# silversixpence-crypto/zk-proof-of-assets

Hardware: AMD Instinct MI355X
Metric: G1-MSM throughput (higher is better)
Workload: dtype u32x8 (254-bit modular integer); 1 GPU; BN254 G1 Pippenger MSM, 2^20 points per GPU, uniform 252-bit scalars, bases (a+i*b)*G resident in HBM (BASELINE.json configs[1]); points_per_gpu=1048576, msms_in_flight=6, form=classic: arbitrary bases, nothing precomputed, checked=not in a plain run (--full checks the known discrete log)

## Files before the change

zk-proof-of-assets_amd/csrc/device_ctx.hpp:

```cpp
#pragma once
#include <hip/hip_runtime.h>
#include <stdint.h>
#include <stdio.h>
#include <stdlib.h>
#include <time.h>
#include <atomic>
#include <condition_variable>
#include <string.h>
#include <exception>
#include <functional>
#include <mutex>
#include <stdexcept>
#include <thread>
#include <string>
#include <vector>

namespace zkpoa {

struct HipError : std::runtime_error {
  explicit HipError(const std::string& s) : std::runtime_error(s) {}
};

struct OomError : HipError {
  explicit OomError(const std::string& s) : HipError(s) {}
// ... 37 lines not shown
    ZK_HIP(e);
    cap = bytes;
  }
  void reset() { off = 0; }
  template <class T>
  T* take(size_t count) {
    size_t bytes = (count * sizeof(T) + 255) & ~size_t(255);
    if (off + bytes > cap) throw HipError("arena overflow (reserve() too small)");
    T* p = reinterpret_cast<T*>(base + off);
    off += bytes;
    return p;
  }
  void release() {
    if (base) (void)hipFree(base);
    base = nullptr;
    cap = off = 0;
  }
};

struct Lane {
  hipStream_t stream = nullptr;
  Arena ws;
  void* pinned = nullptr;
  void* pinned_dev = nullptr;
  size_t pinned_cap = 0;
  std::vector<char> host_sums;
  hipEvent_t ev0 = nullptr, ev1 = nullptr;
  void* scan_scratch = nullptr;
  uint32_t scan_tiles = 0, scan_gen = 0;
  uint32_t scan_poll_limit = 1u << 24, scan_test_withhold = 0;
  static constexpr size_t kFaultBytes = 64;
  volatile uint32_t* fault_word() const { return reinterpret_cast<volatile uint32_t*>(static_cast<char*>(pinned) + pinned_cap); }
  uint32_t* fault_word_dev() const { return reinterpret_cast<uint32_t*>(static_cast<char*>(pinned_dev) + pinned_cap); }
  void init(int level = 0) {
    int lo = 0, hi = 0;
    ZK_HIP(hipDeviceGetStreamPriorityRange(&lo, &hi));
    int prio = level >= 2 ? hi : (level == 1 ? (lo + hi) / 2 : lo);
    ZK_HIP(hipStreamCreateWithPriority(&stream, hipStreamNonBlocking, prio));
    pinned_cap = (1 << 20) - kFaultBytes;
    ZK_HIP(hipHostMalloc(&pinned, pinned_cap + kFaultBytes, hipHostMallocDefault));
    ZK_HIP(hipHostGetDevicePointer(&pinned_dev, pinned, 0));
    memset(static_cast<char*>(pinned) + pinned_cap, 0, kFaultBytes);
    host_sums.assign(pinned_cap + kFaultBytes, 0);
    ZK_HIP(hipEventCreate(&ev0));
    ZK_HIP(hipEventCreate(&ev1));
  }
  void destroy() {
    ws.release();
    if (scan_scratch) (void)hipFree(scan_scratch);
    scan_scratch = nullptr;
    scan_tiles = scan_gen = 0;
    if (pinned) (void)hipHostFree(pinned);
    if (stream) (void)hipStreamDestroy(stream);
    if (ev0) (void)hipEventDestroy(ev0);
    if (ev1) (void)hipEventDestroy(ev1);
    pinned = nullptr;
    stream = nullptr;
    ev0 = ev1 = nullptr;
  }
};

struct DeviceCtx {
  int device = 0;
  int num_cu = 256;
  static constexpr int kLanes = 12;
  static constexpr int kEagerLanes = 5;
  Lane lanes[kLanes];
  std::mutex lazy_mutex_;
  bool ok = false;
  float last_ms[8] = {0, 0, 0, 0, 0, 0, 0, 0};
  std::thread bg_;
  std::mutex bg_mutex_;
  std::condition_variable bg_cv_;
  bool lanes_ready_ = false;
  std::exception_ptr bg_err_;
  hipStream_t copy_stream = nullptr;
  std::function<void(hipStream_t)> after_copy_stream;
  std::function<void()> after_lanes;
  std::mutex copy_mutex_;
  std::condition_variable copy_cv_;
  bool copy_done_ = false;

  void init(int dev) {
    const bool verbose = getenv("ZKPOA_VERBOSE") != nullptr;
    auto now_ms = [] {
      struct timespec ts;
      clock_gettime(CLOCK_MONOTONIC, &ts);
      return ts.tv_sec * 1e3 + ts.tv_nsec / 1e6;
    };
    double t0 = now_ms();
    int count = 0;
// ... 101 lines not shown
```

zk-proof-of-assets_amd/csrc/msm.hip.h:

```cpp
#pragma once
#include "bn254_ec.hip.h"
#include "fq29.hip.h"
#include "device_ctx.hpp"
#include "msm_plan.hpp"
#include <string.h>
#include <chrono>
#include <utility>

namespace zkpoa {

__device__ static const uint32_t kHalfR[8] = {0xf8000000u, 0xa1f0fac9u, 0x3cdcb848u, 0x9419f424u,
                                              0x40c0ac2eu, 0xdc2822dbu, 0x7098d014u, 0x18322739u};

ZK_DEV bool scalar_normalize(uint32_t (&s)[8]) {
  uint32_t bw = 0;
#pragma unroll
  for (int i = 0; i < 8; i++) (void)subb(kHalfR[i], s[i], bw);
  if (!bw) return false;
  uint32_t b2 = 0;
#pragma unroll
  for (int i = 0; i < 8; i++) s[i] = subb(FrParams::P[i], s[i], b2);
  return true;
}

// ... 9 lines not shown
  s[0] = a.x; s[1] = a.y; s[2] = a.z; s[3] = a.w;
  s[4] = b.x; s[5] = b.y; s[6] = b.z; s[7] = b.w;
}

static __global__ __launch_bounds__(256) void msm_density_kernel(const void* __restrict__ scalars, uint64_t n,
                                                                 unsigned long long* __restrict__ out) {
  __shared__ unsigned int acc[kDensityHi - kDensityLo + 1];
  if (threadIdx.x <= (unsigned)(kDensityHi - kDensityLo)) acc[threadIdx.x] = 0;
  __syncthreads();
  uint64_t i = (uint64_t)blockIdx.x * 256u + threadIdx.x;
  uint32_t L = 0;
  if (i < n) {
    uint32_t s[8];
    const uint4* p = reinterpret_cast<const uint4*>(scalars) + 2 * i;
    uint4 a = p[0], b = p[1];
    s[0] = a.x; s[1] = a.y; s[2] = a.z; s[3] = a.w;
    s[4] = b.x; s[5] = b.y; s[6] = b.z; s[7] = b.w;
    (void)scalar_normalize(s);
#pragma unroll
    for (int k = 7; k >= 0; k--)
      if (L == 0 && s[k]) L = 32u * k + (32u - __builtin_clz(s[k]));
  }
  for (int c = kDensityLo; c <= kDensityHi; c++) {
    uint32_t d = (L + c - 1) / c;
#pragma unroll
    for (int o = 32; o > 0; o >>= 1) d += __shfl_xor(d, o);
    if ((threadIdx.x & 63u) == 0 && d) atomicAdd(&acc[c - kDensityLo], d);
  }
  __syncthreads();
  if (threadIdx.x <= (unsigned)(kDensityHi - kDensityLo) && acc[threadIdx.x])
    atomicAdd(&out[threadIdx.x], (unsigned long long)acc[threadIdx.x]);
}

ZK_DEV uint32_t scan_input(const uint32_t* __restrict__ in, uint32_t idx, uint32_t n, int mode, uint32_t K,
                           uint32_t& raw) {
  if (idx >= n) {
    raw = 0;
    return 0;
  }
  uint32_t x = in[idx];
  if (mode == 3) x = in[idx + 1] - x;
  raw = x;
  if (mode == 0) return x;
  if (mode == 3 && x <= 1) return 0;
  return (x + K - 1) / K;
}
constexpr int kScanBlock = 256;
constexpr int kScanItems = 8;
constexpr int kScanTile = kScanBlock * kScanItems;

ZK_DEV uint32_t block_exclusive_scan(uint32_t v, uint32_t* lds, uint32_t& total) {
  uint32_t lane = threadIdx.x & 63u, wave = threadIdx.x >> 6;
  uint32_t x = v;
#pragma unroll
  for (int o = 1; o < 64; o <<= 1) {
    uint32_t y = __shfl_up(x, o);
    if (lane >= (uint32_t)o) x += y;
  }
  if (lane == 63) lds[wave] = x;
  __syncthreads();
  uint32_t base = 0, tot = 0;
#pragma unroll
  for (int k = 0; k < kScanBlock / 64; k++) {
    uint32_t t = lds[k];
    if ((uint32_t)k < wave) base += t;
    tot += t;
  }
  __syncthreads();
  total = tot;
  return base + x - v;
}

static __global__ __launch_bounds__(kScanBlock) void scan_reduce_kernel(const uint32_t* __restrict__ in, uint32_t n, int mode,
                                                                 uint32_t K, uint32_t* __restrict__ block_sums,
                                                                 uint32_t* __restrict__ max_out) {
  __shared__ uint32_t lds[8];
  uint32_t base = blockIdx.x * kScanTile + threadIdx.x * kScanItems;
  uint32_t sum = 0, mx = 0;
// ... 137 lines not shown
  if (lane == 0) scan_status_store(&status[tile], tag2 | (running + aggregate));
  return running;
}

static __global__ __launch_bounds__(kScanBlock) void scan_pair_kernel(ScanPair a, uint64_t* __restrict__ status_a,
                                                                      uint64_t* __restrict__ status_b,
                                                                      uint32_t* __restrict__ tickets, uint32_t gen,
                                                                      uint32_t ntiles, ScanGuard guard) {
  __shared__ uint32_t lds[8];
  __shared__ uint32_t s_tile, s_pre_a, s_pre_b;
  __shared__ uint32_t s_hist[kMaxPieceLenPlan + 1];
  if (threadIdx.x == 0) s_tile = atomicAdd(&tickets[0], 1u);
  if (a.hist)
    for (uint32_t i = threadIdx.x; i <= a.hist_K; i += kScanBlock) s_hist[i] = 0;
  __syncthreads();
  const uint32_t tile = s_tile;
  const uint32_t base = tile * kScanTile + threadIdx.x * kScanItems;
  const bool two = a.mode_b >= 0;
  uint32_t va[kScanItems], vb[kScanItems];
  uint32_t sum_a = 0, sum_b = 0, mx = 0;
#pragma unroll
  for (int k = 0; k < kScanItems; k++) {
    uint32_t raw;
    va[k] = scan_input(a.in, base + k, a.n, a.mode_a, a.K_a, raw);
    sum_a += va[k];
    mx = raw > mx ? raw : mx;
    if (a.hist && raw) {
      const uint32_t full = raw / a.hist_K, rem = raw - full * a.hist_K;
      if (full) atomicAdd(&s_hist[a.hist_K], full);
      if (rem) atomicAdd(&s_hist[rem], 1u);
    }
    vb[k] = 0;
    if (two) {
      if (a.mode_b == 0) vb[k] = raw;
      else if (a.mode_b == 3 && raw <= 1) vb[k] = 0;
      else vb[k] = (raw + a.K_b - 1) / a.K_b;
      sum_b += vb[k];
    }
  }
  uint32_t tot_a, tot_b = 0;
  uint32_t ex_a = block_exclusive_scan(sum_a, lds, tot_a);
  uint32_t ex_b = two ? block_exclusive_scan(sum_b, lds, tot_b) : 0;
  if (threadIdx.x < 64) {
    uint32_t pa = scan_look_back(status_a, tile, tot_a, gen, guard);
    uint32_t pb = two ? scan_look_back(status_b, tile, tot_b, gen, guard) : 0;
    if (threadIdx.x == 0) {
      s_pre_a = pa;
      s_pre_b = pb;
    }
  }
  __syncthreads();
  ex_a += s_pre_a;
  ex_b += s_pre_b;
#pragma unroll
  for (int k = 0; k < kScanItems; k++) {
    const uint32_t idx = base + k;
    if (idx < a.n) {
      a.out_a[idx] = ex_a;
      if (two) a.out_b[idx] = ex_b;
    }
    ex_a += va[k];
    ex_b += vb[k];
  }
  if (tile == ntiles - 1 && threadIdx.x == kScanBlock - 1) {
    a.out_a[a.n] = ex_a;
    if (a.total_a) *a.total_a = ex_a;
    if (two) {
      a.out_b[a.n] = ex_b;
      if (a.total_b) *a.total_b = ex_b;
// ... 69 lines not shown
ZK_DEV uint32_t find_bucket(const uint32_t* __restrict__ po, uint32_t nb, uint32_t t) {
  uint32_t lo = 0, hi = nb;
  while (hi - lo > 1) {
    uint32_t mid = (lo + hi) >> 1;
    if (po[mid] <= t) lo = mid; else hi = mid;
  }
  return lo;
}

}
#include "msm_sort.hip.h"
namespace zkpoa {

constexpr uint32_t kMaxPieceLen = 512;
static_assert(kMaxPieceLen == kMaxPieceLenPlan, "the plan, the scans' LDS histogram and the piece ordering share one bound");

constexpr uint32_t kPiecesPerThread = 8;
static __global__ __launch_bounds__(256) void msm_piece_hist_kernel(const uint32_t* __restrict__ cnt0, uint32_t TB,
                                                                    uint32_t K0, uint32_t* __restrict__ len_hist) {
  __shared__ uint32_t h[kMaxPieceLen + 1];
  for (uint32_t i = threadIdx.x; i <= K0; i += 256u) h[i] = 0;
  __syncthreads();
  const uint32_t b = blockIdx.x * 256u + threadIdx.x;
  const uint32_t x = b < TB ? cnt0[b] : 0u;
  if (x) {
    const uint32_t full = x / K0, rem = x - full * K0;
    if (full) atomicAdd(&h[K0], full);
    if (rem) atomicAdd(&h[rem], 1u);
  }
  __syncthreads();
  for (uint32_t i = threadIdx.x; i <= K0; i += 256u)
    if (h[i]) atomicAdd(&len_hist[i], h[i]);
}
static __global__ __launch_bounds__(256) void msm_piece_order_kernel(const uint32_t* __restrict__ cnt0,
                                                                     const uint32_t* __restrict__ po1, uint32_t TB,
                                                                     uint32_t K0, const uint32_t* __restrict__ len_hist,
                                                                     uint32_t* __restrict__ cursor,
                                                                     uint32_t* __restrict__ pbkt,
                                                                     uint32_t* __restrict__ order) {
  __shared__ uint32_t base[kMaxPieceLen + 2];
  __shared__ uint32_t h[kMaxPieceLen + 1];
  __shared__ uint32_t wsum[4];
  uint32_t tid = threadIdx.x;
  uint32_t v0 = 0, v1 = 0, v2 = 0;
  uint32_t r0 = 3 * tid, r1 = 3 * tid + 1, r2 = 3 * tid + 2;
  if (r0 <= kMaxPieceLen) v0 = len_hist[kMaxPieceLen - r0];
  if (r1 <= kMaxPieceLen) v1 = len_hist[kMaxPieceLen - r1];
  if (r2 <= kMaxPieceLen) v2 = len_hist[kMaxPieceLen - r2];
  uint32_t tot;
  uint32_t ex = block_exclusive_scan(v0 + v1 + v2, wsum, tot);
  if (r0 <= kMaxPieceLen) base[kMaxPieceLen - r0] = ex;
  if (r1 <= kMaxPieceLen) base[kMaxPieceLen - r1] = ex + v0;
  if (r2 <= kMaxPieceLen) base[kMaxPieceLen - r2] = ex + v0 + v1;
  for (uint32_t i = tid; i <= kMaxPieceLen; i += 256u) h[i] = 0;
  __syncthreads();
  const uint32_t total = po1[TB];
  uint32_t len[kPiecesPerThread], local[kPiecesPerThread];
#pragma unroll
  for (uint32_t k = 0; k < kPiecesPerThread; k++) {
    const uint32_t t = (blockIdx.x * kPiecesPerThread + k) * 256u + tid;
    len[k] = 0;
    local[k] = 0;
    if (t < total) {
      const uint32_t b = find_bucket(po1, TB, t);
      const uint32_t j = t - po1[b];
      uint32_t l = cnt0[b] - j * K0;
      if (l > K0) l = K0;
      pbkt[t] = b;
      len[k] = l;
      local[k] = atomicAdd(&h[l], 1u);
    }
  }
  __syncthreads();
  for (uint32_t i = tid; i <= kMaxPieceLen; i += 256u) {
    uint32_t c = h[i];
    if (c) h[i] = atomicAdd(&cursor[i], c);
  }
  __syncthreads();
#pragma unroll
  for (uint32_t k = 0; k < kPiecesPerThread; k++) {
    const uint32_t t = (blockIdx.x * kPiecesPerThread + k) * 256u + tid;
    if (t < total) order[base[len[k]] + h[len[k]] + local[k]] = t;
  }
}

#if defined(ZKPOA_G1_LIMB32)
constexpr bool kG1Limb29 = false;
#else
constexpr bool kG1Limb29 = true;
#endif
ZK_DEV XYZZ<Fq> xyzz_from_words_3q(const uint32_t* w) {
  XYZZ<Fq> r;
#pragma unroll
  for (int i = 0; i < 8; i++) {
    r.x.l[i] = w[i];
    r.y.l[i] = w[8 + i];
    r.zz.l[i] = w[16 + i];
    r.zzz.l[i] = w[24 + i];
  }
  r.x = Fq::reduce_2p(r.x);
  r.y = Fq::reduce_2p(r.y);
  r.zz = Fq::reduce_2p(r.zz);
  r.zzz = Fq::reduce_2p(r.zzz);
  return r;
}
ZK_DEV bool g1piece29_result(const G1Piece29& s, XYZZ<Fq>& out) {
  uint32_t w[32];
  g1piece29_finish(s, w);
  out = xyzz_from_words_3q(w);
  return s.empty || !out.zz.is_zero();
}

struct G1Sum29 {
  Xyzz29S p;
  bool inf;
// ... 373 lines not shown
template <class F, bool Packed = false, bool WireOut = false>
static __global__ __launch_bounds__(64, kRedWaves<Packed>) void msm_bit_tree_sum_kernel(const void* __restrict__ X, uint32_t E,
                                                                     uint32_t logS, uint32_t logRows, uint32_t nbits,
                                                                     uint32_t S_out, void* __restrict__ Y) {
  extern __shared__ __attribute__((aligned(16))) char lds_raw[];
  const uint32_t g = blockIdx.y / nbits, b = blockIdx.y % nbits, grp = g & 1u;
  const uint32_t cnt = grp ? (1u << logS) : (1u << logRows);
  msm_tree_run<F, Packed, WireOut>(X, (size_t)g * E, cnt, grp, (int)b, Y, (size_t)blockIdx.y * S_out + blockIdx.x, lds_raw);
}
template <class F, bool Packed = false, bool WireOut = false>
static __global__ __launch_bounds__(64, kRedWaves<Packed>) void msm_tree_sum_kernel(const void* __restrict__ X, uint32_t S, uint32_t S_out,
                                                           void* __restrict__ Y) {
  extern __shared__ __attribute__((aligned(16))) char lds_raw[];
  const uint32_t w = blockIdx.y;
  msm_tree_run<F, Packed, WireOut>(X, (size_t)w * S, S, 0u, -1, Y, (size_t)w * S_out + blockIdx.x, lds_raw);
}

template <class F>
struct MsmSizes {
  static constexpr size_t kAffine = 2 * FieldBytes<F>::N;
  static constexpr size_t kXyzz = 4 * FieldBytes<F>::N;
};

static __global__ __launch_bounds__(256) void msm_to_host_kernel(const uint4* __restrict__ src, uint4* __restrict__ dst,
                                                                 uint32_t n16) {
  for (uint32_t i = blockIdx.x * 256u + threadIdx.x; i < n16; i += gridDim.x * 256u) dst[i] = src[i];
}
inline void msm_read_back(Lane& lane, const void* d_src, size_t bytes) {
  if (bytes > lane.pinned_cap) throw HipError("msm: read-back larger than the pinned staging area");
  const uint32_t n16 = (uint32_t)((bytes + 15) / 16);
  const uint32_t grid = n16 > 4096 ? 16u : (n16 + 255) / 256;
  hipLaunchKernelGGL(msm_to_host_kernel, dim3(grid ? grid : 1), dim3(256), 0, lane.stream, (const uint4*)d_src,
                     (uint4*)lane.pinned_dev, n16);
  ZK_HIP(hipStreamSynchronize(lane.stream));
  lane_check_fault(lane);
}

inline void lane_scan(Lane& lane, const ScanPair& a, uint32_t* block_sums) {
  if (!scan_three_kernel()) return scan_pair(lane, a);
  scan_u32(lane.stream, a.in, a.n, a.mode_a, a.K_a, a.out_a, block_sums, a.total_a, a.max_out);
  if (a.mode_b >= 0) scan_u32(lane.stream, a.in, a.n, a.mode_b, a.K_b, a.out_b, block_sums, a.total_b, nullptr);
  if (a.hist)
    hipLaunchKernelGGL(msm_piece_hist_kernel, dim3((a.n + 255) / 256), dim3(256), 0, lane.stream, a.in, a.n, a.hist_K, a.hist);
}

struct ArenaCount {
  size_t off = 0;
  template <class T> T* take(size_t count) { return off += (count * sizeof(T) + 255) & ~size_t(255), nullptr; }
};
template <class Layout>
inline size_t msm_layout_bytes(const MsmPlan& p) {
  ArenaCount count;
  Layout().carve(count, p);
  return count.off;
}
template <class Layout>
inline Layout msm_carve(Arena& ws, const MsmPlan& p) {
  Layout m;
  const size_t start = ws.off;
  m.carve(ws, p);
  if (ws.off - start != msm_layout_bytes<Layout>(p)) throw HipError("msm: internal: workspace layout and its size disagree");
  return m;
}
inline size_t msm_piece_cap(const MsmPlan& p) { return (size_t)p.n * p.W / p.K0 + p.TB + 1; }

struct MsmSortLayout {
// ... 47 lines not shown
  char* buckets = nullptr;
  char *P1 = nullptr, *P2 = nullptr;
  size_t p1_cap = 0, p2_cap = 0;
  char* X = nullptr;
  char *Y1 = nullptr, *Y2 = nullptr;
  template <class Taker>
  void carve(Taker& ws, const MsmPlan& p) {
    constexpr size_t kXyzz = MsmSizes<F>::kXyzz;
    const size_t E = (size_t)1 << p.logS, sums = (size_t)2 * p.Wb * msm_reduce_bits(p.logS);
    po_b = ws.template take<uint32_t>(p.TB + 1);
    po_c = ws.template take<uint32_t>(p.TB + 1);
    block_sums = ws.template take<uint32_t>(p.TB / kScanTile + 2);
    misc = ws.template take<uint32_t>(16);
    buckets = ws.template take<char>((size_t)p.TB * kXyzz);
    p1_cap = msm_piece_cap(p);
    p2_cap = p1_cap / 2 + 1;
    P1 = ws.template take<char>(p1_cap * kXyzz);
    P2 = ws.template take<char>(p2_cap * kXyzz);
    X = ws.template take<char>(2 * p.Wb * E * kXyzz);
    Y1 = ws.template take<char>((E + 255) / 256 * sums * kXyzz);
    Y2 = ws.template take<char>((E + 255) / 256 * sums * kXyzz);
  }
};

inline size_t msm_sort_workspace_bytes(const MsmPlan& p) { return msm_layout_bytes<MsmSortLayout>(p) + (1 << 12) - 256; }
template <class F>
inline size_t msm_accum_workspace_bytes(const MsmPlan& p) { return msm_layout_bytes<MsmAccumLayout<F>>(p) + (1 << 12); }

template <class F, bool Packed = false, class Scan>
inline void msm_reduce_levels(hipStream_t st, uint32_t TB, uint32_t K, const uint32_t* po_in, uint32_t* po_b,
                              uint32_t* po_c, char* Pin, size_t cap_in, char* Pout, size_t cap_out, uint64_t max_items,
                              uint64_t total_in, void* buckets, Scan scan) {
  uint32_t* po_out = po_b;
  while (max_items > 1) {
    uint64_t bound = total_in / 2 + 1;
    if (bound > cap_out) throw HipError("msm: level buffer too small");
    scan(po_in, po_out);
    hipLaunchKernelGGL((msm_accumN_kernel<F, Packed>), dim3((uint32_t)((bound + 255) / 256)), dim3(256), 0, st, (const void*)Pin,
                       po_in, (const uint32_t*)po_out, TB, K, buckets, (void*)Pout);
    max_items = (max_items + K - 1) / K;
    total_in = bound;
    po_in = po_out;
    po_out = (po_out == po_b) ? po_c : po_b;
    std::swap(Pin, Pout);
    std::swap(cap_in, cap_out);
  }
}

struct MsmSorted {
  MsmPlan p;
  MsmSortLayout m;
  uint32_t total1 = 0;
  uint32_t total_entries = 0;
  uint32_t max_count = 0;
};

inline void lane_reserve(Lane& lane, size_t need) {
  if (lane.ws.cap < need) {
    ZK_HIP(hipStreamSynchronize(lane.stream));
    const auto t0 = std::chrono::steady_clock::now();
    lane.ws.reserve(need);
    const double ms = std::chrono::duration<double, std::milli>(std::chrono::steady_clock::now() - t0).count();
    if (ms > 20.0 && getenv("ZKPOA_VERBOSE"))
      fprintf(stderr, "zkpoa:   lane workspace grows to %.2f GB: hipFree + hipMalloc %.1f ms\n", need / 1e9, ms);
  }
}

inline MsmSorted msm_sort_phase(Lane& lane, const void* d_scalars, const MsmRequest& req,
                                size_t (*extra)(const MsmPlan&), bool sync_at_end = false) {
  MsmSorted sr;
  sr.p = msm_make_plan(req);
  const MsmPlan& p = sr.p;
  if ((uint64_t)p.n * p.W + p.TB >= 0xffff0000ull) throw HipError("msm: n * windows exceeds the 32-bit entry index");
  if (p.merged && (uint64_t)p.n * p.W >= 0x80000000ull) throw HipError("msm: n * windows exceeds the fixed-base entry index");
  hipStream_t st = lane.stream;
  lane_reserve(lane, msm_sort_workspace_bytes(p) + (extra ? extra(p) : 0));
  lane.ws.reset();
  const SortPlan sp = make_sort_plan(p.ne, p.Wb, p.c);
  const MsmSortLayout& m = sr.m = msm_carve<MsmSortLayout>(lane.ws, p);
  ZK_HIP(hipMemsetAsync(m.counts, 0, m.zero_bytes, st));
  static const bool no_sparse = [] {
    const char* e = getenv("ZKPOA_NO_SPARSE");
    return e && *e == '1';
  }();
  const bool sparse = p.sparse && !no_sparse;
  uint32_t* digits = sparse ? nullptr : m.digits();
  uint2* elist = sparse ? m.elist : nullptr;
  uint32_t* pre = sparse ? m.pre : nullptr;
  const uint32_t nblk = (p.n + 255) / 256;
  if (p.n && !sparse) hipLaunchKernelGGL(msm_digits_kernel, dim3(nblk), dim3(256), 0, st, d_scalars, p.n, p.c, p.W, digits);
  if (sparse) {
    const uint32_t per_wg = kEntriesThreads * kEntriesPerThread;
    hipLaunchKernelGGL(msm_entries_kernel, dim3((p.n + per_wg - 1) / per_wg), dim3(kEntriesThreads), 0, st, d_scalars, p.n,
                       p.c, p.W, elist, m.misc + 8);
    hipLaunchKernelGGL(msm_entries_finish_kernel, dim3(1), dim3(1), 0, st, (const uint32_t*)(m.misc + 8), sp.CH, pre, pre + 4);
  }
  for (uint32_t l = 0; l < sp.npass; l++) {
    const bool first = l == 0 && !sparse, last = l + 1 == sp.npass;
    const uint2* in = l == 0 ? (const uint2*)elist : m.ebuf[(l - 1) & 1];
    uint2* out = last ? nullptr : m.ebuf[l & 1];
    const uint32_t* in_off = l == 0 ? (const uint32_t*)pre : m.seg_off[l - 1];
    const uint32_t* tpo = l == 0 ? (const uint32_t*)(pre ? pre + 4 : nullptr) : m.seg_tpo[l - 1];
    uint32_t* out_cnt = last ? m.counts : m.seg_cnt[l];
    uint32_t* out_off = last ? m.off0 : m.seg_off[l];
    const dim3 grid = first ? dim3(sp.chunks0, sp.W) : dim3((uint32_t)sp.tasks_max[l]);
    if (p.n) {
      if (first)
        hipLaunchKernelGGL((msm_sort_count_kernel<true>), grid, dim3(256), 0, st, sp, l, (const uint32_t*)digits, in,
                           in_off, tpo, out_cnt, m.base[l]);
      else
        hipLaunchKernelGGL((msm_sort_count_kernel<false>), grid, dim3(256), 0, st, sp, l, (const uint32_t*)digits, in,
                           in_off, tpo, out_cnt, m.base[l]);
    }
    lane_scan(lane,
              last ? ScanPair{m.counts, p.TB, 0, 0, m.off0, m.misc + 0, 1, p.K0, m.po_a, m.misc + 2, m.misc + 1, m.len_hist, p.K0}
                   : ScanPair{m.seg_cnt[l], sp.segs[l + 1], 0, 0, m.seg_off[l], m.misc + 4 + 2 * l, 1, sp.CH, m.seg_tpo[l],
                              m.misc + 5 + 2 * l, nullptr},
              m.block_sums);
    if (p.n) {
#define ZK_SORT_SCATTER(F_, L_)                                                                                       \
  hipLaunchKernelGGL((msm_sort_scatter_kernel<F_, L_>), grid, dim3(256), 0, st, sp, l, (const uint32_t*)digits, in,  \
                     in_off, tpo, (const uint32_t*)out_off, (const uint32_t*)m.base[l], out, m.sorted)
      if (first && last) ZK_SORT_SCATTER(true, true);
      else if (first) ZK_SORT_SCATTER(true, false);
      else if (last) ZK_SORT_SCATTER(false, true);
      else ZK_SORT_SCATTER(false, false);
#undef ZK_SORT_SCATTER
    }
  }
  uint32_t* hb = reinterpret_cast<uint32_t*>(lane.pinned);
  msm_read_back(lane, m.misc, 16);
  sr.total_entries = hb[0];
  sr.max_count = hb[1];
  sr.total1 = hb[2];
  if (sr.total1) {
    const uint32_t per_block = 256u * kPiecesPerThread;
    hipLaunchKernelGGL(msm_piece_order_kernel, dim3((sr.total1 + per_block - 1) / per_block), dim3(256), 0, st,
                       (const uint32_t*)m.counts, (const uint32_t*)m.po_a, p.TB, p.K0, (const uint32_t*)m.len_hist,
                       m.len_cursor(), m.pbkt, m.order);
  }
  if (sync_at_end) ZK_HIP(hipStreamSynchronize(st));
  return sr;
}

template <class F>
inline void msm_accum_phase(Lane& lane, const MsmSorted& sr, const void* d_bases, void* window_sums_host,
                            bool own_arena, float* accum_ms = nullptr) {
  const MsmPlan& p = sr.p;
  hipStream_t st = lane.stream;
  if (!own_arena) {
    lane_reserve(lane, msm_accum_workspace_bytes<F>(p));
    lane.ws.reset();
  }
  const MsmAccumLayout<F> m = msm_carve<MsmAccumLayout<F>>(lane.ws, p);
  const uint32_t E = 1u << p.logS, S1 = (E + 255) / 256;
  const uint32_t nbits = msm_reduce_bits(p.logS), sums = 2u * p.Wb * nbits;

  if (accum_ms) ZK_HIP(hipEventRecord(lane.ev0, st));
  if (sr.total1) {
    const uint32_t pgrid = (sr.total1 + 255) / 256;
    hipLaunchKernelGGL((msm_accum0_kernel<F>), dim3(pgrid), dim3(256), 0, st, d_bases, (const uint32_t*)sr.m.sorted,
                       (const uint32_t*)sr.m.counts, (const uint32_t*)sr.m.off0, (const uint32_t*)sr.m.po_a,
                       (const uint32_t*)sr.m.order, (const uint32_t*)sr.m.pbkt, p.TB, p.K0, (void*)m.buckets, (void*)m.P1);
  }
  if (accum_ms) ZK_HIP(hipEventRecord(lane.ev1, st));
  auto scan = [&](auto* in, auto* out) { lane_scan(lane, ScanPair{in, p.TB, 3, p.K, out, m.misc + 3, -1}, m.block_sums); };
  constexpr bool kPacked = kPackedSums<F>;
  constexpr size_t kLds = RedOps<F, kPacked>::kLds;
  msm_reduce_levels<F, kPacked>(st, p.TB, p.K, sr.m.po_a, m.po_b, m.po_c, m.P1, m.p1_cap, m.P2, m.p2_cap,
                       ((uint64_t)sr.max_count + p.K0 - 1) / p.K0, sr.total1, m.buckets, scan);
  {
    uint32_t log_parts = msm_reduce_log_parts(p.logRows, p.logS, p.Wb);
    uint64_t threads = ((uint64_t)p.Wb << log_parts) * ((1u << p.logRows) + E);
    hipLaunchKernelGGL((msm_bucket_sums_kernel<F, kPacked>), dim3((uint32_t)((threads + 255) / 256)), dim3(256),
                       256 * kLds, st, (const void*)m.buckets, (const uint32_t*)sr.m.counts, p.Wb, p.Nb, p.logS,
                       p.logRows, log_parts, E, (void*)m.X);
  }
  char *cur = m.Y1, *next = m.Y2;
  if (S1 == 1)
    hipLaunchKernelGGL((msm_bit_tree_sum_kernel<F, kPacked, true>), dim3(S1, sums), dim3(64), 64 * kLds, st,
                       (const void*)m.X, E, p.logS, p.logRows, nbits, S1, (void*)cur);
  else
    hipLaunchKernelGGL((msm_bit_tree_sum_kernel<F, kPacked, false>), dim3(S1, sums), dim3(64), 64 * kLds, st,
                       (const void*)m.X, E, p.logS, p.logRows, nbits, S1, (void*)cur);
  for (uint32_t S = S1; S > 1; S = (S + 255) / 256, std::swap(cur, next)) {
    const uint32_t S_out = (S + 255) / 256;
    if (S_out == 1)
      hipLaunchKernelGGL((msm_tree_sum_kernel<F, kPacked, true>), dim3(S_out, sums), dim3(64), 64 * kLds, st,
                         (const void*)cur, S, S_out, (void*)next);
    else
      hipLaunchKernelGGL((msm_tree_sum_kernel<F, kPacked, false>), dim3(S_out, sums), dim3(64), 64 * kLds, st,
                         (const void*)cur, S, S_out, (void*)next);
  }
  msm_read_back(lane, cur, (size_t)sums * MsmSizes<F>::kXyzz);
  ZK_HIP(hipGetLastError());
  memcpy(window_sums_host, lane.pinned, (size_t)sums * MsmSizes<F>::kXyzz);
  if (accum_ms) ZK_HIP(hipEventElapsedTime(accum_ms, lane.ev0, lane.ev1));
}

struct MsmTable {
  void* d = nullptr;
  uint64_t n = 0;
  uint32_t c = 0, W = 0;
  size_t bytes = 0;
};

template <class F>
static __global__ __launch_bounds__(256) void msm_table_chain_kernel(const void* __restrict__ bases, uint64_t i0,
                                                                      uint64_t cnt, uint32_t c, uint32_t W,
                                                                      void* __restrict__ scratch) {
  uint64_t t = (uint64_t)blockIdx.x * 256u + threadIdx.x;
  if (t >= cnt) return;
  XYZZ<F> acc = XYZZ<F>::from_affine(load_affine<F>(bases, i0 + t));
  for (uint32_t j = 0; j < W; j++) {
    store_xyzz(scratch, (size_t)j * cnt + t, acc);
    if (j + 1 < W)
      for (uint32_t k = 0; k < c; k++) acc = xyzz_dbl(acc);
  }
}

template <class F>
static __global__ __launch_bounds__(256) void msm_table_affine_kernel(const void* __restrict__ scratch,
                                                                       void* __restrict__ prefix, uint64_t i0,
                                                                       uint64_t cnt, uint64_t n, uint32_t W,
                                                                       void* __restrict__ table) {
  uint64_t t = (uint64_t)blockIdx.x * 256u + threadIdx.x;
  if (t >= cnt) return;
// ... 57 lines not shown
    ZK_HIP(hipMalloc(&prefix, (size_t)(n < slab ? (n ? n : 1) : slab) * t.W * FieldBytes<F>::N));
    for (uint64_t off = 0; off < n; off += slab) {
      const uint64_t cnt = n - off < slab ? n - off : slab;
      hipLaunchKernelGGL((msm_table_chain_kernel<F>), dim3((uint32_t)((cnt + 255) / 256)), dim3(256), 0, st, d_bases, off,
                         cnt, t.c, t.W, scratch);
      hipLaunchKernelGGL((msm_table_affine_kernel<F>), dim3((uint32_t)((cnt + 255) / 256)), dim3(256), 0, st,
                         (const void*)scratch, prefix, off, cnt, n, t.W, t.d);
    }
    ZK_HIP(hipStreamSynchronize(st));
    ZK_HIP(hipGetLastError());
  } catch (...) {
    if (scratch) (void)hipFree(scratch);
    if (prefix) (void)hipFree(prefix);
    (void)hipFree(t.d);
    throw;
  }
  (void)hipFree(scratch);
  (void)hipFree(prefix);
  return t;
}

inline void msm_table_free(MsmTable& t) {
  if (t.d) (void)hipFree(t.d);
  t = MsmTable();
}

template <class F>
inline MsmPlan msm_device(Lane& lane, const void* d_bases, const void* d_scalars, const MsmRequest& req,
                          void* window_sums_host, float* accum_ms = nullptr, const MsmTable* table = nullptr,
                          uint32_t* entries = nullptr) {
  if (req.merged != (table != nullptr)) throw HipError("msm: internal: a merged request and its table go together");
  if (table && (table->n != req.n || (int)table->c != req.c))
    throw HipError("msm: the fixed-base table was built for another base array");
  MsmSorted sr = msm_sort_phase(lane, d_scalars, req, &msm_accum_workspace_bytes<F>);
  msm_accum_phase<F>(lane, sr, table ? table->d : d_bases, window_sums_host, true, accum_ms);
  if (entries) *entries = sr.total_entries;
  return sr.p;
}

}
```

zk-proof-of-assets_amd/csrc/msm_run.hip.h:

```cpp
#pragma once
#include "msm.hip.h"

#include <chrono>
#include <thread>
#include "zkpoa_internal.hpp"

namespace zkpoa {
template <class F, class HF>
void msm_run(zkpoa_context* ctx, int lane_id, const void* d_bases, const void* d_scalars, uint64_t n, uint8_t* out,
             float* ms2, const MsmTable* table = nullptr, const double* density = nullptr) {
  if (lane_id) ctx->dev.wait_lanes();
  ctx->dev.ensure_lane(lane_id);
  Lane& lane = ctx->dev.lanes[lane_id];
  std::vector<char>& wsums = lane.host_sums;
  XYZZ<HF> total = XYZZ<HF>::inf();
  float tot_ms = 0, acc_sum = 0;
  uint64_t done = 0, adds = 0;
  uint32_t hold_waits = 0;
  do {
    const uint64_t max_pts = ctx->msm_points_limit(lane_id);
    if (table && (n > max_pts || table->n != n)) table = nullptr;
    const uint64_t cnt = n - done < max_pts ? n - done : max_pts;
    float acc_ms = 0;
    uint32_t entries = 0;
// ... 17 lines not shown
        fprintf(stderr, "zkpoa:   lane %d: %s for %llu points at once; continuing with at most %llu\n", lane_id, e.what(),
                (unsigned long long)cnt, (unsigned long long)ctx->msm_points_limit(lane_id));
      continue;
    }
    adds += entries;
    ZK_HIP(hipEventRecord(ctx->ev_b[lane_id], lane.stream));
    ZK_HIP(hipEventSynchronize(ctx->ev_b[lane_id]));
    float tot = 0;
    ZK_HIP(hipEventElapsedTime(&tot, ctx->ev_a[lane_id], ctx->ev_b[lane_id]));
    tot_ms += tot;
    acc_sum += acc_ms;
    XYZZ<HF> r = h_combine_windows<HF>(wsums.data(), p.Wb, p.c, p.logS);
    if (done == 0) total = r;
    else xyzz_add(total, r);
    done += cnt;
  } while (done < n);
  if (ms2) {
    ms2[0] = tot_ms;
    ms2[1] = acc_sum;
  }
  ctx->lane_adds[lane_id] = (double)adds;
  h_affine_to_bytes<HF>(h_to_affine(total), out);
}


template <class F, class HF>
void msm_accum_run(zkpoa_context* ctx, int lane_id, const MsmSorted& sr, bool own_arena, const void* d_bases,
                   uint8_t* out, float* ms2) {
  if (lane_id) ctx->dev.wait_lanes();
  Lane& lane = ctx->dev.lanes[lane_id];
  std::vector<char>& wsums = lane.host_sums;
  float acc_ms = 0;
  ZK_HIP(hipEventRecord(ctx->ev_a[lane_id], lane.stream));
  msm_accum_phase<F>(lane, sr, d_bases, wsums.data(), own_arena, &acc_ms);
  ZK_HIP(hipEventRecord(ctx->ev_b[lane_id], lane.stream));
  ZK_HIP(hipEventSynchronize(ctx->ev_b[lane_id]));
  float tot = 0;
  ZK_HIP(hipEventElapsedTime(&tot, ctx->ev_a[lane_id], ctx->ev_b[lane_id]));
  if (ms2) {
    ms2[0] = tot;
    ms2[1] = acc_ms;
  }
  ctx->lane_adds[lane_id] = (double)sr.total_entries;
  XYZZ<HF> r = h_combine_windows<HF>(wsums.data(), sr.p.Wb, sr.p.c, sr.p.logS);
  h_affine_to_bytes<HF>(h_to_affine(r), out);
}

}
```

zk-proof-of-assets_amd/csrc/msm_sort.hip.h:

```cpp
#pragma once
#include "bn254_field.hip.h"

namespace zkpoa {

constexpr uint32_t kSortMaxBits = 8;
constexpr uint32_t kSortMaxBins = 1u << kSortMaxBits;
constexpr uint32_t kSortEpt = 8;
constexpr uint32_t kSortTile = 256u * kSortEpt;
constexpr uint32_t kSortMaxPasses = 3;

struct SortPlan {
  uint32_t n, W, c, Nb;
  uint32_t npass;
  uint32_t bits[kSortMaxPasses];
  uint32_t rem[kSortMaxPasses];
  uint32_t segs[kSortMaxPasses + 1];
  uint32_t CH;
  uint32_t chunks0;
  uint64_t tasks_max[kSortMaxPasses];
};

inline SortPlan make_sort_plan(uint32_t n, uint32_t W, uint32_t c) {
  SortPlan s{};
  s.n = n; s.W = W; s.c = c; s.Nb = 1u << (c - 1);
// ... 8 lines not shown
    left -= s.bits[l];
    s.segs[l + 1] = s.segs[l] << s.bits[l];
  }
  s.CH = 8u * kSortTile;
  s.chunks0 = n ? (n + s.CH - 1) / s.CH : 1;
  s.tasks_max[0] = (uint64_t)s.chunks0 * W;
  for (uint32_t l = 1; l < s.npass; l++) s.tasks_max[l] = ((uint64_t)n * W) / s.CH + s.segs[l] + 1;
  return s;
}

ZK_DEV uint32_t lds_count_rank(uint32_t* lds, uint32_t key, bool valid) {
  const uint32_t lane = threadIdx.x & 63u;
  unsigned long long vm = __ballot(valid);
  uint32_t rank = 0;
  bool done = !valid;
  if (vm) {
    int first = __ffsll((long long)vm) - 1;
    uint32_t k0 = __shfl(key, first);
    unsigned long long m = __ballot(valid && key == k0);
    if (valid && key == k0) {
      uint32_t base = 0;
      if ((int)lane == first) base = atomicAdd(&lds[k0], (uint32_t)__popcll(m));
      base = __shfl(base, first);
      rank = base + (uint32_t)__popcll(m & ((1ull << lane) - 1ull));
      done = true;
    }
  }
  if (!done) rank = atomicAdd(&lds[key], 1u);
  return rank;
}

static __global__ __launch_bounds__(256) void msm_digits_kernel(const void* __restrict__ scalars, uint32_t n,
                                                                uint32_t c, uint32_t W,
                                                                uint32_t* __restrict__ digits) {
  uint32_t i = blockIdx.x * 256u + threadIdx.x;
  if (i >= n) return;
  uint32_t s[8];
  load_scalar(scalars, i, s);
  bool neg = scalar_normalize(s);
  const uint32_t Nb = 1u << (c - 1), mask = (1u << c) - 1u;
  uint32_t carry = 0;
  for (uint32_t w = 0; w < W; w++) {
    uint32_t d = (s[0] & mask) + carry;
    scalar_shr(s, c);
    carry = d > Nb ? 1u : 0u;
    uint32_t mag = carry ? (mask + 1u - d) : d;
    bool sign = (carry != 0) != neg;
    digits[(size_t)w * n + i] = mag | ((sign && mag) ? 0x80000000u : 0u);
  }
}

constexpr uint32_t kEntriesThreads = 1024, kEntriesPerThread = 2;
constexpr uint32_t kEntriesStage = 8192;
template <class Fn>
ZK_DEV void for_nonzero_digits(uint32_t (&s)[8], bool neg, uint32_t c, uint32_t W, Fn f) {
  const uint32_t Nb = 1u << (c - 1), mask = (1u << c) - 1u;
  uint32_t carry = 0;
  for (uint32_t w = 0; w < W; w++) {
    const uint32_t d = (s[0] & mask) + carry;
    scalar_shr(s, c);
    carry = d > Nb ? 1u : 0u;
    const uint32_t mag = carry ? (mask + 1u - d) : d;
    if (mag) f(w, mag, (carry != 0) != neg);
  }
}
static __global__ __launch_bounds__(kEntriesThreads) void msm_entries_kernel(const void* __restrict__ scalars, uint32_t n,
                                                                            uint32_t c, uint32_t W, uint2* __restrict__ out,
                                                                            uint32_t* __restrict__ counter) {
// ... 208 lines not shown
```

zk-proof-of-assets_amd/csrc/setup.hip:

```cpp
#include "abc.hip.h"
#include "msm.hip.h"
#include "hooks.hip.h"
#include "pairing.hpp"
#include "phase2_dev.hip.h"
#include "setup_common.hip.h"
#include "zkpoa_internal.hpp"

#include <mutex>

using namespace zkpoa;

namespace {

static __global__ __launch_bounds__(256) void setup_hist_kernel(const uint32_t* __restrict__ sig,
                                                                const uint32_t* __restrict__ pidx,
                                                                const void* __restrict__ coefs, uint32_t nnz,
                                                                uint32_t n_signals, uint32_t n_points,
                                                                uint32_t* __restrict__ counts, uint32_t* __restrict__ flags) {
  uint32_t e = blockIdx.x * 256u + threadIdx.x;
  if (e >= nnz) return;
  uint32_t s = sig[e];
  uint32_t k[8];
  load_scalar(coefs, e, k);
  uint32_t bw = 0;
// ... 163 lines not shown
  constexpr size_t X = MsmSizes<F>::kXyzz;
  DevBuf counts((size_t)S * 4), off(((size_t)S + 1) * 4), po_b(((size_t)S + 1) * 4), po_c(((size_t)S + 1) * 4),
      block_sums(((size_t)S / kScanTile + 2) * 4), misc(64), order((size_t)(N ? N : 1) * 4), buckets((size_t)S * X),
      items((size_t)(N ? N : 1) * X), items2(((size_t)N / 2 + 2) * X), by_len((size_t)(N ? N : 1) * 4), len_hist(1024 * 4);
  uint32_t* m = reinterpret_cast<uint32_t*>(misc.p);
  ZK_HIP(hipMemsetAsync(counts.p, 0, (size_t)S * 4, st));
  ZK_HIP(hipMemsetAsync(misc.p, 0, 64, st));
  ZK_HIP(hipMemsetAsync(buckets.p, 0, (size_t)S * X, st));
  const uint32_t grid = (N + 255) / 256;
  if (N)
    hipLaunchKernelGGL(setup_hist_kernel, dim3(grid), dim3(256), 0, st, d_sig, d_pidx, d_coefs, N, S, (uint32_t)n_points,
                       (uint32_t*)counts.p, m);
  scan_u32(st, (const uint32_t*)counts.p, S, 0, 0, (uint32_t*)off.p, (uint32_t*)block_sums.p, m + 1, m + 2);
  msm_read_back(lane, m, 16);
  const uint32_t* hb = reinterpret_cast<const uint32_t*>(lane.pinned);
  const uint32_t flags = hb[0], total = hb[1], max_seg = hb[2];
  if (flags & 1u) throw HipError("setup_accumulate: signal or point index out of range");
  if (flags & 2u) throw HipError("setup_accumulate: coefficient is not a field element (>= r)");
  if (total != N) throw HipError("setup_accumulate: internal: histogram does not add up");
  if (N) {
    ZK_HIP(hipMemsetAsync(counts.p, 0, (size_t)S * 4, st));
    hipLaunchKernelGGL(setup_scatter_kernel, dim3(grid), dim3(256), 0, st, d_sig, N, (const uint32_t*)off.p,
                       (uint32_t*)counts.p, (uint32_t*)order.p);
    uint32_t* lh = reinterpret_cast<uint32_t*>(len_hist.p);
    ZK_HIP(hipMemsetAsync(len_hist.p, 0, 1024 * 4, st));
    hipLaunchKernelGGL(setup_len_hist_kernel, dim3(grid), dim3(256), 0, st, d_coefs, (const uint32_t*)order.p, N, lh);
    scan_u32(st, lh, 256, 0, 0, lh + 256, (uint32_t*)block_sums.p, m + 3, nullptr);
    hipLaunchKernelGGL(setup_len_scatter_kernel, dim3(grid), dim3(256), 0, st, d_coefs, (const uint32_t*)order.p, N,
                       (const uint32_t*)(lh + 256), lh + 520, (uint32_t*)by_len.p);
    hipLaunchKernelGGL((setup_mul_kernel<F>), dim3(grid), dim3(256), 0, st, d_points, d_coefs, d_pidx, d_sig,
                       (const uint32_t*)order.p, (const uint32_t*)by_len.p, (const uint32_t*)off.p, N, buckets.p, items.p);
  }
  const uint32_t K = 4;
  auto scan = [&](const uint32_t* in, uint32_t* out) { scan_u32(st, in, S, 3, K, out, (uint32_t*)block_sums.p, m + 3, nullptr); };
  msm_reduce_levels<F>(st, S, K, (const uint32_t*)off.p, (uint32_t*)po_b.p, (uint32_t*)po_c.p, (char*)items.p, N ? N : 1,
                       (char*)items2.p, (size_t)N / 2 + 2, max_seg, N, buckets.p, scan);
  hipLaunchKernelGGL((xyzz_to_affine_kernel<F>), dim3((S + 255) / 256), dim3(256), 0, st, (const void*)buckets.p, d_out,
                     (uint64_t)S);
  ZK_HIP(hipStreamSynchronize(st));
  ZK_HIP(hipGetLastError());
}

}

extern "C" int zkpoa_setup_accumulate(zkpoa_context* ctx, int group, const void* d_points, uint64_t n_points,
                                      const void* d_coefs, const uint32_t* d_point_index, const uint32_t* d_signal,
                                      uint64_t nnz, uint64_t n_signals, void* d_out) {
  ZK_API_BEGIN(ctx)
  if (group != 1 && group != 2) throw HipError("setup_accumulate: group must be 1 (G1) or 2 (G2)");
  if ((nnz && (!d_points || !d_coefs || !d_point_index || !d_signal)) || (n_signals && !d_out))
    throw HipError("setup_accumulate: null pointer");
  if (group == 1) setup_accumulate<Fq>(ctx, d_points, n_points, d_coefs, d_point_index, d_signal, nnz, n_signals, d_out);
  else setup_accumulate<Fq2>(ctx, d_points, n_points, d_coefs, d_point_index, d_signal, nnz, n_signals, d_out);
  ZK_API_END(ctx)
}

namespace {

void dev_check_coords(zkpoa_context* ctx, const void* d, uint64_t count32, const char* what) {
  if (!count32) return;
  hipStream_t st = ctx->dev.lanes[0].stream;
  DevBuf flag(64);
  ZK_HIP(hipMemsetAsync(flag.p, 0, 64, st));
  hipLaunchKernelGGL((range_check_kernel<FqParams>), dim3((uint32_t)((count32 + 255) / 256)), dim3(256), 0, st, d, count32,
                     (uint32_t*)flag.p);
  uint32_t bad = 0;
  ZK_HIP(hipMemcpyAsync(&bad, flag.p, 4, hipMemcpyDeviceToHost, st));
// ... 613 lines not shown
```

Baseline: 641.7 million pts/s.

## Defer sort totals read-back and drop host syncs in MSM pipeline

```diff
diff --git a/zk-proof-of-assets_amd/csrc/device_ctx.hpp b/zk-proof-of-assets_amd/csrc/device_ctx.hpp
--- a/zk-proof-of-assets_amd/csrc/device_ctx.hpp
+++ b/zk-proof-of-assets_amd/csrc/device_ctx.hpp
@@ -93,18 +93,25 @@
   static constexpr size_t kFaultBytes = 64;
   volatile uint32_t* fault_word() const { return reinterpret_cast<volatile uint32_t*>(static_cast<char*>(pinned) + pinned_cap); }
   uint32_t* fault_word_dev() const { return reinterpret_cast<uint32_t*>(static_cast<char*>(pinned_dev) + pinned_cap); }
+  static constexpr size_t kTotalsBytes = 64;
+  volatile uint32_t* totals() const {
+    return reinterpret_cast<volatile uint32_t*>(static_cast<char*>(pinned) + pinned_cap + kFaultBytes);
+  }
+  uint32_t* totals_dev() const { return reinterpret_cast<uint32_t*>(static_cast<char*>(pinned_dev) + pinned_cap + kFaultBytes); }
+  hipEvent_t ev_totals = nullptr;
   void init(int level = 0) {
     int lo = 0, hi = 0;
     ZK_HIP(hipDeviceGetStreamPriorityRange(&lo, &hi));
     int prio = level >= 2 ? hi : (level == 1 ? (lo + hi) / 2 : lo);
     ZK_HIP(hipStreamCreateWithPriority(&stream, hipStreamNonBlocking, prio));
-    pinned_cap = (1 << 20) - kFaultBytes;
-    ZK_HIP(hipHostMalloc(&pinned, pinned_cap + kFaultBytes, hipHostMallocDefault));
+    pinned_cap = (1 << 20) - kFaultBytes - kTotalsBytes;
+    ZK_HIP(hipHostMalloc(&pinned, pinned_cap + kFaultBytes + kTotalsBytes, hipHostMallocDefault));
     ZK_HIP(hipHostGetDevicePointer(&pinned_dev, pinned, 0));
-    memset(static_cast<char*>(pinned) + pinned_cap, 0, kFaultBytes);
+    memset(static_cast<char*>(pinned) + pinned_cap, 0, kFaultBytes + kTotalsBytes);
     host_sums.assign(pinned_cap + kFaultBytes, 0);
     ZK_HIP(hipEventCreate(&ev0));
     ZK_HIP(hipEventCreate(&ev1));
+    ZK_HIP(hipEventCreate(&ev_totals));
   }
   void destroy() {
     ws.release();
@@ -115,9 +122,10 @@
     if (stream) (void)hipStreamDestroy(stream);
     if (ev0) (void)hipEventDestroy(ev0);
     if (ev1) (void)hipEventDestroy(ev1);
+    if (ev_totals) (void)hipEventDestroy(ev_totals);
     pinned = nullptr;
     stream = nullptr;
-    ev0 = ev1 = nullptr;
+    ev0 = ev1 = ev_totals = nullptr;
   }
 };
 
diff --git a/zk-proof-of-assets_amd/csrc/msm.hip.h b/zk-proof-of-assets_amd/csrc/msm.hip.h
--- a/zk-proof-of-assets_amd/csrc/msm.hip.h
+++ b/zk-proof-of-assets_amd/csrc/msm.hip.h
@@ -65,6 +65,13 @@
     atomicAdd(&out[threadIdx.x], (unsigned long long)acc[threadIdx.x]);
 }
 
+ZK_DEV uint32_t scan_transform(uint32_t x, int mode, uint32_t K) {
+  if (mode == 0) return x;
+  if (mode >= 3 && x <= 1) return 0;
+  const uint32_t p = (x + K - 1) / K;
+  if (mode != 4) return p;
+  return p <= 1 ? 0 : (p + K - 1) / K;
+}
 ZK_DEV uint32_t scan_input(const uint32_t* __restrict__ in, uint32_t idx, uint32_t n, int mode, uint32_t K,
                            uint32_t& raw) {
   if (idx >= n) {
@@ -72,11 +79,9 @@
     return 0;
   }
   uint32_t x = in[idx];
-  if (mode == 3) x = in[idx + 1] - x;
+  if (mode >= 3) x = in[idx + 1] - x;
   raw = x;
-  if (mode == 0) return x;
-  if (mode == 3 && x <= 1) return 0;
-  return (x + K - 1) / K;
+  return scan_transform(x, mode, K);
 }
 constexpr int kScanBlock = 256;
 constexpr int kScanItems = 8;
@@ -280,9 +285,7 @@
     }
     vb[k] = 0;
     if (two) {
-      if (a.mode_b == 0) vb[k] = raw;
-      else if (a.mode_b == 3 && raw <= 1) vb[k] = 0;
-      else vb[k] = (raw + a.K_b - 1) / a.K_b;
+      vb[k] = scan_transform(raw, a.mode_b, a.K_b);
       sum_b += vb[k];
     }
   }
@@ -418,15 +421,33 @@
   for (uint32_t i = threadIdx.x; i <= K0; i += 256u)
     if (h[i]) atomicAdd(&len_hist[i], h[i]);
 }
+struct MsmTotals {
+  const uint32_t* misc;
+  uint32_t* host;
+  const uint32_t* fault;
+  uint32_t* po1_total;
+};
 static __global__ __launch_bounds__(256) void msm_piece_order_kernel(const uint32_t* __restrict__ cnt0,
                                                                      const uint32_t* __restrict__ po1, uint32_t TB,
                                                                      uint32_t K0, const uint32_t* __restrict__ len_hist,
                                                                      uint32_t* __restrict__ cursor,
                                                                      uint32_t* __restrict__ pbkt,
-                                                                     uint32_t* __restrict__ order) {
+                                                                     uint32_t* __restrict__ order, uint32_t cap,
+                                                                     MsmTotals tot_out) {
   __shared__ uint32_t base[kMaxPieceLen + 2];
   __shared__ uint32_t h[kMaxPieceLen + 1];
   __shared__ uint32_t wsum[4];
+  const uint32_t total = po1[TB];
+  if (blockIdx.x == 0) {
+    if (threadIdx.x == 0) {
+      tot_out.host[0] = tot_out.misc[0];
+      tot_out.host[1] = tot_out.misc[1];
+      tot_out.host[2] = tot_out.misc[2];
+      if (__hip_atomic_load(tot_out.fault, __ATOMIC_RELAXED, __HIP_MEMORY_SCOPE_SYSTEM)) *tot_out.po1_total = 0;
+    }
+  } else if (blockIdx.x * (256u * kPiecesPerThread) >= total) {
+    return;
+  }
   uint32_t tid = threadIdx.x;
   uint32_t v0 = 0, v1 = 0, v2 = 0;
   uint32_t r0 = 3 * tid, r1 = 3 * tid + 1, r2 = 3 * tid + 2;
@@ -440,14 +461,13 @@
   if (r2 <= kMaxPieceLen) base[kMaxPieceLen - r2] = ex + v0 + v1;
   for (uint32_t i = tid; i <= kMaxPieceLen; i += 256u) h[i] = 0;
   __syncthreads();
-  const uint32_t total = po1[TB];
   uint32_t len[kPiecesPerThread], local[kPiecesPerThread];
 #pragma unroll
   for (uint32_t k = 0; k < kPiecesPerThread; k++) {
     const uint32_t t = (blockIdx.x * kPiecesPerThread + k) * 256u + tid;
     len[k] = 0;
     local[k] = 0;
-    if (t < total) {
+    if (t < total && t < cap) {
       const uint32_t b = find_bucket(po1, TB, t);
       const uint32_t j = t - po1[b];
       uint32_t l = cnt0[b] - j * K0;
@@ -466,7 +486,10 @@
 #pragma unroll
   for (uint32_t k = 0; k < kPiecesPerThread; k++) {
     const uint32_t t = (blockIdx.x * kPiecesPerThread + k) * 256u + tid;
-    if (t < total) order[base[len[k]] + h[len[k]] + local[k]] = t;
+    if (t < total && t < cap) {
+      const uint32_t pos = base[len[k]] + h[len[k]] + local[k];
+      if (pos < cap) order[pos] = t;
+    }
   }
 }
 
@@ -906,6 +929,15 @@
   const uint32_t grid = n16 > 4096 ? 16u : (n16 + 255) / 256;
   hipLaunchKernelGGL(msm_to_host_kernel, dim3(grid ? grid : 1), dim3(256), 0, lane.stream, (const uint4*)d_src,
                      (uint4*)lane.pinned_dev, n16);
+  ZK_HIP(hipStreamSynchronize(lane.stream));
+  lane_check_fault(lane);
+}
+
+inline void msm_sums_fit(const Lane& lane, size_t bytes) {
+  if (bytes > lane.pinned_cap) throw HipError("msm: read-back larger than the pinned staging area");
+}
+inline void msm_sums_wait(Lane& lane, size_t bytes) {
+  msm_sums_fit(lane, bytes);
   ZK_HIP(hipStreamSynchronize(lane.stream));
   lane_check_fault(lane);
 }
@@ -1019,10 +1051,12 @@
                               uint32_t* po_c, char* Pin, size_t cap_in, char* Pout, size_t cap_out, uint64_t max_items,
                               uint64_t total_in, void* buckets, Scan scan) {
   uint32_t* po_out = po_b;
-  while (max_items > 1) {
+  const bool two = (max_items + K - 1) / K > 1;
+  for (uint32_t level = 1; max_items > 1; level++) {
     uint64_t bound = total_in / 2 + 1;
     if (bound > cap_out) throw HipError("msm: level buffer too small");
-    scan(po_in, po_out);
+    if (level == 1) scan(po_in, po_b, two ? po_c : (uint32_t*)nullptr);
+    else if (level > 2) scan(po_in, po_out, (uint32_t*)nullptr);
     hipLaunchKernelGGL((msm_accumN_kernel<F, Packed>), dim3((uint32_t)((bound + 255) / 256)), dim3(256), 0, st, (const void*)Pin,
                        po_in, (const uint32_t*)po_out, TB, K, buckets, (void*)Pout);
     max_items = (max_items + K - 1) / K;
@@ -1040,7 +1074,22 @@
   uint32_t total1 = 0;
   uint32_t total_entries = 0;
   uint32_t max_count = 0;
+  bool deferred = false;
 };
+
+inline void msm_sort_resolve(Lane& lane, MsmSorted& sr) {
+  if (!sr.deferred) return;
+  ZK_HIP(hipEventSynchronize(lane.ev_totals));
+  if (*lane.fault_word()) {
+    ZK_HIP(hipStreamSynchronize(lane.stream));
+    lane_check_fault(lane);
+  }
+  volatile uint32_t* hb = lane.totals();
+  sr.total_entries = hb[0];
+  sr.max_count = hb[1];
+  sr.total1 = hb[2];
+  sr.deferred = false;
+}
 
 inline void lane_reserve(Lane& lane, size_t need) {
   if (lane.ws.cap < need) {
@@ -1054,7 +1103,7 @@
 }
 
 inline MsmSorted msm_sort_phase(Lane& lane, const void* d_scalars, const MsmRequest& req,
-                                size_t (*extra)(const MsmPlan&), bool sync_at_end = false) {
+                                size_t (*extra)(const MsmPlan&), bool sync_at_end = false, bool defer = false) {
   MsmSorted sr;
   sr.p = msm_make_plan(req);
   const MsmPlan& p = sr.p;
@@ -1065,7 +1114,6 @@
   lane.ws.reset();
   const SortPlan sp = make_sort_plan(p.ne, p.Wb, p.c);
   const MsmSortLayout& m = sr.m = msm_carve<MsmSortLayout>(lane.ws, p);
-  ZK_HIP(hipMemsetAsync(m.counts, 0, m.zero_bytes, st));
   static const bool no_sparse = [] {
     const char* e = getenv("ZKPOA_NO_SPARSE");
     return e && *e == '1';
@@ -1075,7 +1123,11 @@
   uint2* elist = sparse ? m.elist : nullptr;
   uint32_t* pre = sparse ? m.pre : nullptr;
   const uint32_t nblk = (p.n + 255) / 256;
-  if (p.n && !sparse) hipLaunchKernelGGL(msm_digits_kernel, dim3(nblk), dim3(256), 0, st, d_scalars, p.n, p.c, p.W, digits);
+  if (p.n && !sparse)
+    hipLaunchKernelGGL(msm_digits_kernel, dim3(nblk), dim3(256), 0, st, d_scalars, p.n, p.c, p.W, digits,
+                       reinterpret_cast<uint4*>(m.counts), (uint32_t)(m.zero_bytes / 16));
+  else
+    ZK_HIP(hipMemsetAsync(m.counts, 0, m.zero_bytes, st));
   if (sparse) {
     const uint32_t per_wg = kEntriesThreads * kEntriesPerThread;
     hipLaunchKernelGGL(msm_entries_kernel, dim3((p.n + per_wg - 1) / per_wg), dim3(kEntriesThreads), 0, st, d_scalars, p.n,
@@ -1115,25 +1167,25 @@
 #undef ZK_SORT_SCATTER
     }
   }
-  uint32_t* hb = reinterpret_cast<uint32_t*>(lane.pinned);
-  msm_read_back(lane, m.misc, 16);
-  sr.total_entries = hb[0];
-  sr.max_count = hb[1];
-  sr.total1 = hb[2];
-  if (sr.total1) {
-    const uint32_t per_block = 256u * kPiecesPerThread;
-    hipLaunchKernelGGL(msm_piece_order_kernel, dim3((sr.total1 + per_block - 1) / per_block), dim3(256), 0, st,
+  {
+    const uint32_t per_block = 256u * kPiecesPerThread, cap = (uint32_t)msm_piece_cap(p);
+    hipLaunchKernelGGL(msm_piece_order_kernel, dim3((cap + per_block - 1) / per_block), dim3(256), 0, st,
                        (const uint32_t*)m.counts, (const uint32_t*)m.po_a, p.TB, p.K0, (const uint32_t*)m.len_hist,
-                       m.len_cursor(), m.pbkt, m.order);
-  }
+                       m.len_cursor(), m.pbkt, m.order, cap,
+                       MsmTotals{m.misc, lane.totals_dev(), lane.fault_word_dev(), m.po_a + p.TB});
+    ZK_HIP(hipEventRecord(lane.ev_totals, st));
+    sr.deferred = true;
+  }
+  if (!defer) msm_sort_resolve(lane, sr);
   if (sync_at_end) ZK_HIP(hipStreamSynchronize(st));
   return sr;
 }
 
 template <class F>
-inline void msm_accum_phase(Lane& lane, const MsmSorted& sr, const void* d_bases, void* window_sums_host,
+inline void msm_accum_phase(Lane& lane, MsmSorted& sr, const void* d_bases, void* window_sums_host,
                             bool own_arena, float* accum_ms = nullptr) {
   const MsmPlan& p = sr.p;
+  if (sr.deferred && !own_arena) throw HipError("msm: internal: a deferred sort is accumulated on its own lane");
   hipStream_t st = lane.stream;
   if (!own_arena) {
     lane_reserve(lane, msm_accum_workspace_bytes<F>(p));
@@ -1142,16 +1194,20 @@
   const MsmAccumLayout<F> m = msm_carve<MsmAccumLayout<F>>(lane.ws, p);
   const uint32_t E = 1u << p.logS, S1 = (E + 255) / 256;
   const uint32_t nbits = msm_reduce_bits(p.logS), sums = 2u * p.Wb * nbits;
+  msm_sums_fit(lane, (size_t)sums * MsmSizes<F>::kXyzz);
 
   if (accum_ms) ZK_HIP(hipEventRecord(lane.ev0, st));
-  if (sr.total1) {
-    const uint32_t pgrid = (sr.total1 + 255) / 256;
+  if (sr.deferred || sr.total1) {
+    const uint32_t pgrid = (uint32_t)(((sr.deferred ? msm_piece_cap(p) : (size_t)sr.total1) + 255) / 256);
     hipLaunchKernelGGL((msm_accum0_kernel<F>), dim3(pgrid), dim3(256), 0, st, d_bases, (const uint32_t*)sr.m.sorted,
                        (const uint32_t*)sr.m.counts, (const uint32_t*)sr.m.off0, (const uint32_t*)sr.m.po_a,
                        (const uint32_t*)sr.m.order, (const uint32_t*)sr.m.pbkt, p.TB, p.K0, (void*)m.buckets, (void*)m.P1);
   }
   if (accum_ms) ZK_HIP(hipEventRecord(lane.ev1, st));
-  auto scan = [&](auto* in, auto* out) { lane_scan(lane, ScanPair{in, p.TB, 3, p.K, out, m.misc + 3, -1}, m.block_sums); };
+  msm_sort_resolve(lane, sr);
+  auto scan = [&](const uint32_t* in, uint32_t* out, uint32_t* out2) {
+    lane_scan(lane, ScanPair{in, p.TB, 3, p.K, out, m.misc + 3, out2 ? 4 : -1, p.K, out2, m.misc + 4, nullptr}, m.block_sums);
+  };
   constexpr bool kPacked = kPackedSums<F>;
   constexpr size_t kLds = RedOps<F, kPacked>::kLds;
   msm_reduce_levels<F, kPacked>(st, p.TB, p.K, sr.m.po_a, m.po_b, m.po_c, m.P1, m.p1_cap, m.P2, m.p2_cap,
@@ -1166,7 +1222,7 @@
   char *cur = m.Y1, *next = m.Y2;
   if (S1 == 1)
     hipLaunchKernelGGL((msm_bit_tree_sum_kernel<F, kPacked, true>), dim3(S1, sums), dim3(64), 64 * kLds, st,
-                       (const void*)m.X, E, p.logS, p.logRows, nbits, S1, (void*)cur);
+                       (const void*)m.X, E, p.logS, p.logRows, nbits, S1, lane.pinned_dev);
   else
     hipLaunchKernelGGL((msm_bit_tree_sum_kernel<F, kPacked, false>), dim3(S1, sums), dim3(64), 64 * kLds, st,
                        (const void*)m.X, E, p.logS, p.logRows, nbits, S1, (void*)cur);
@@ -1174,12 +1230,12 @@
     const uint32_t S_out = (S + 255) / 256;
     if (S_out == 1)
       hipLaunchKernelGGL((msm_tree_sum_kernel<F, kPacked, true>), dim3(S_out, sums), dim3(64), 64 * kLds, st,
-                         (const void*)cur, S, S_out, (void*)next);
+                         (const void*)cur, S, S_out, lane.pinned_dev);
     else
       hipLaunchKernelGGL((msm_tree_sum_kernel<F, kPacked, false>), dim3(S_out, sums), dim3(64), 64 * kLds, st,
                          (const void*)cur, S, S_out, (void*)next);
   }
-  msm_read_back(lane, cur, (size_t)sums * MsmSizes<F>::kXyzz);
+  msm_sums_wait(lane, (size_t)sums * MsmSizes<F>::kXyzz);
   ZK_HIP(hipGetLastError());
   memcpy(window_sums_host, lane.pinned, (size_t)sums * MsmSizes<F>::kXyzz);
   if (accum_ms) ZK_HIP(hipEventElapsedTime(accum_ms, lane.ev0, lane.ev1));
@@ -1303,7 +1359,7 @@
   if (req.merged != (table != nullptr)) throw HipError("msm: internal: a merged request and its table go together");
   if (table && (table->n != req.n || (int)table->c != req.c))
     throw HipError("msm: the fixed-base table was built for another base array");
-  MsmSorted sr = msm_sort_phase(lane, d_scalars, req, &msm_accum_workspace_bytes<F>);
+  MsmSorted sr = msm_sort_phase(lane, d_scalars, req, &msm_accum_workspace_bytes<F>, false, true);
   msm_accum_phase<F>(lane, sr, table ? table->d : d_bases, window_sums_host, true, accum_ms);
   if (entries) *entries = sr.total_entries;
   return sr.p;
diff --git a/zk-proof-of-assets_amd/csrc/msm_run.hip.h b/zk-proof-of-assets_amd/csrc/msm_run.hip.h
--- a/zk-proof-of-assets_amd/csrc/msm_run.hip.h
+++ b/zk-proof-of-assets_amd/csrc/msm_run.hip.h
@@ -73,7 +73,8 @@
   std::vector<char>& wsums = lane.host_sums;
   float acc_ms = 0;
   ZK_HIP(hipEventRecord(ctx->ev_a[lane_id], lane.stream));
-  msm_accum_phase<F>(lane, sr, d_bases, wsums.data(), own_arena, &acc_ms);
+  MsmSorted done = sr;
+  msm_accum_phase<F>(lane, done, d_bases, wsums.data(), own_arena, &acc_ms);
   ZK_HIP(hipEventRecord(ctx->ev_b[lane_id], lane.stream));
   ZK_HIP(hipEventSynchronize(ctx->ev_b[lane_id]));
   float tot = 0;
diff --git a/zk-proof-of-assets_amd/csrc/msm_sort.hip.h b/zk-proof-of-assets_amd/csrc/msm_sort.hip.h
--- a/zk-proof-of-assets_amd/csrc/msm_sort.hip.h
+++ b/zk-proof-of-assets_amd/csrc/msm_sort.hip.h
@@ -64,8 +64,10 @@
 
 static __global__ __launch_bounds__(256) void msm_digits_kernel(const void* __restrict__ scalars, uint32_t n,
                                                                 uint32_t c, uint32_t W,
-                                                                uint32_t* __restrict__ digits) {
+                                                                uint32_t* __restrict__ digits, uint4* __restrict__ zero,
+                                                                uint32_t zero16) {
   uint32_t i = blockIdx.x * 256u + threadIdx.x;
+  for (uint32_t z = i; z < zero16; z += gridDim.x * 256u) zero[z] = make_uint4(0, 0, 0, 0);
   if (i >= n) return;
   uint32_t s[8];
   load_scalar(scalars, i, s);
diff --git a/zk-proof-of-assets_amd/csrc/setup.hip b/zk-proof-of-assets_amd/csrc/setup.hip
--- a/zk-proof-of-assets_amd/csrc/setup.hip
+++ b/zk-proof-of-assets_amd/csrc/setup.hip
@@ -219,7 +219,10 @@
                        (const uint32_t*)order.p, (const uint32_t*)by_len.p, (const uint32_t*)off.p, N, buckets.p, items.p);
   }
   const uint32_t K = 4;
-  auto scan = [&](const uint32_t* in, uint32_t* out) { scan_u32(st, in, S, 3, K, out, (uint32_t*)block_sums.p, m + 3, nullptr); };
+  auto scan = [&](const uint32_t* in, uint32_t* out, uint32_t* out2) {
+    scan_u32(st, in, S, 3, K, out, (uint32_t*)block_sums.p, m + 3, nullptr);
+    if (out2) scan_u32(st, in, S, 4, K, out2, (uint32_t*)block_sums.p, m + 3, nullptr);
+  };
   msm_reduce_levels<F>(st, S, K, (const uint32_t*)off.p, (uint32_t*)po_b.p, (uint32_t*)po_c.p, (char*)items.p, N ? N : 1,
                        (char*)items2.p, (size_t)N / 2 + 2, max_seg, N, buckets.p, scan);
   hipLaunchKernelGGL((xyzz_to_affine_kernel<F>), dim3((S + 255) / 256), dim3(256), 0, st, (const void*)buckets.p, d_out,
```

Result: no change. 645.4 million pts/s, median of 6 (+0.6%).
